# JiaruiFeng/KP-GNN

Hardware: AMD Instinct MI355X
Metric: graphs/sec KP-GIN fwd+bwd, ZINC-12k K=8 L=8 h=104 (higher is better)
Workload: dtype f32; 1 GPU; ZINC-12k-shaped synthetic molecules, KPGINPlus K=8 L=8 h=104 kernel=spd geometric combine, fwd+bwd+Adam, L1 loss; global_batch=2048, nodes_per_batch=47450, khop_edges_per_batch=1018372, active_pairs_per_batch=1018372, parallelism=dp1, launch=hipGraph replay of fwd+bwd, batches=4 pre-staged batches cycled

## Files before the change

### include/kpgnn.h

```cpp
#ifndef KPGNN_H_
#define KPGNN_H_

#include <stddef.h>
#include <stdint.h>

#ifdef __cplusplus
extern "C" {
#endif

#define KPGNN_ABI_VERSION 1

#define KPGNN_OK 0
#define KPGNN_EINVAL (-1)
#define KPGNN_EHIP (-2)
#define KPGNN_ELIMIT (-3)

typedef void* kpgnn_stream_t;

int kpgnn_abi_version(void);
const char* kpgnn_last_error(void);

int kpgnn_device_info(int* cu_count, int* lds_bytes_per_block, int* wavefront, char* arch, int arch_len);


// ... 44 lines not shown
    int32_t* rowptr_dst; int32_t* col_dst; uint16_t* code_dst;
    int32_t* rowptr_src; int32_t* col_src; uint16_t* code_src;
    int64_t* batch;
    int32_t* node_src;
    int32_t nodes_per_tile; int32_t* tile_ptr; uint32_t* tile_pack;
    int32_t* ent_node_ptr;
    int32_t num_prefix; int32_t* prefix_ptr; uint32_t* prefix_pack; int32_t* prefix_scratch;
    int32_t n_node_rows; kpgnn_row_gather node_rows[8];
    int32_t n_graph_rows; kpgnn_row_gather graph_rows[8];
} kpgnn_collate_desc;

int kpgnn_collate(const kpgnn_collate_desc* d, kpgnn_stream_t stream);

int kpgnn_regression_loss(const float* score, const float* y, int64_t n, int32_t kind, float* loss, float* dscore,
                          kpgnn_stream_t stream);

int kpgnn_score_head_fwd(const float* pooled, const float* w, const float* bias, int64_t G, int32_t D, float* score,
                         kpgnn_stream_t stream);
int kpgnn_score_head_bwd(const float* pooled, const float* w, const float* dscore, int64_t G, int32_t D, float* dpooled,
                         float* dw, float* db, kpgnn_stream_t stream);

int kpgnn_adam_step(float* param, const float* grad, float* exp_avg, float* exp_avg_sq, int64_t n, int64_t step,
                    double lr, double beta1, double beta2, double eps, double weight_decay, kpgnn_stream_t stream);

int kpgnn_adam_step_device(float* param, const float* grad, float* exp_avg, float* exp_avg_sq, int64_t n, int64_t* state,
                           double lr, double beta1, double beta2, double eps, double weight_decay, kpgnn_stream_t stream);

int kpgnn_multi_copy(int32_t count, const float* const* src, float* const* dst, const int64_t* numel, kpgnn_stream_t stream);

typedef struct kpgnn_reduce_job {
    const float* slab; int32_t nslab; int64_t elems;
    float* out[4]; int64_t n_out[4];
} kpgnn_reduce_job;
int kpgnn_reduce_jobs(const kpgnn_reduce_job* jobs, int32_t count, kpgnn_stream_t stream);

enum { KPGNN_STORE_F32 = 0, KPGNN_STORE_BF16 = 1 };

enum { KPGNN_MATH_AUTO = 0, KPGNN_MATH_F32 = 1 };

enum {
    KPGNN_MODE_GIN = 0,
    KPGNN_MODE_GINPLUS = 1,
    KPGNN_MODE_GCN = 2,
    KPGNN_MODE_SUM = 3
};

typedef struct kpgnn_agg_fwd_desc {
    int32_t N, K, D;
    int32_t K_csr;
    int32_t mode;
    int32_t n_code0, n_codek;
    int32_t use_tables;
    const int32_t* rowptr;
    const int32_t* col;
    const uint16_t* code;
    const float* dis;
    const float* x;
    int64_t x_sn, x_sk;
    const float* table0;
    const float* tablek;
    const float* periph;
    int64_t p_sn, p_sk;
    const float* eps;
    float* out;
    int64_t o_sn, o_sk;
    float* pre;
    const float* theta;
    float* hout;
    const float* xbias;
    const float* ptab;
    const int32_t* uid;
    int64_t uid_stride;
    const float* x_slot[16];
    int32_t n_dict;
    const float* alphas;
    int32_t storage;
    const int32_t* n_dyn;
    const int32_t* graph_ptr; int32_t num_graphs; int32_t max_graph_nodes;
    const float* hinit;
    const float* hinit2;
} kpgnn_agg_fwd_desc;

int kpgnn_aggregate_fwd(const kpgnn_agg_fwd_desc* d, kpgnn_stream_t stream);

typedef struct kpgnn_agg_bwd_desc {
    int32_t N, K, D, K_csr, mode, n_code0, n_codek, use_tables;
    const int32_t* rowptr_src;
    const int32_t* col_src;
    const uint16_t* code_src;
    const float* dis;
    const float* g;
    int64_t g_sn, g_sk;
    const float* eps;
    float* gx;
    int64_t gx_sn, gx_sk;
    float* gtable0;
    float* gtablek;
    float* gx_slot[16];
    uint32_t accumulate_mask;
    int32_t storage;
    const int32_t* n_dyn;
} kpgnn_agg_bwd_desc;

int kpgnn_aggregate_bwd(const kpgnn_agg_bwd_desc* d, kpgnn_stream_t stream);

typedef struct kpgnn_table_grad_desc {
    int32_t N, K, D, nodes_per_tile, n_code0, n_codek;
    int32_t n_dict, dict_src;
    const int32_t* tile_ptr;
    const uint32_t* tile_pack;
    const float* g;
    int64_t g_sn, g_sk;
    const int32_t* uid;
    int64_t uid_stride;
    const float* theta;
    const float* gh;
    float* gtable0;
    float* gtablek;
    float* gdict;
    void* workspace;
    size_t workspace_bytes;
    int32_t kernel;
    const uint32_t* dict_pack;
    int32_t dict_pack_K;
    const float* extra_slab;
    int32_t extra_nslab;
    int64_t extra_elems;
    float* extra_out;
    int32_t storage;
    const float* fuse_pre;
    const float* fuse_ptab;
    const int32_t* fuse_uid;
    int64_t fuse_uid_stride;
    int32_t fuse_n_dict;
    float* fuse_g;
    float* fuse_gtheta;
    const float* fuse_alphas;
    float* fuse_galphas;
    void* fuse_workspace;
    size_t fuse_workspace_bytes;
    int32_t accumulate_dict;
    const kpgnn_reduce_job* pending;
    const int32_t* n_dyn;
    int32_t max_multiplicity;
} kpgnn_table_grad_desc;

size_t kpgnn_table_grad_workspace_bytes(int32_t N, int32_t K, int32_t D, int32_t nodes_per_tile,
                                        int32_t n_code0, int32_t n_codek, int32_t n_dict);
int kpgnn_table_grad(const kpgnn_table_grad_desc* d, kpgnn_stream_t stream);
size_t kpgnn_table_grad_fuse_workspace_bytes(int32_t K, int32_t D);
int kpgnn_dict_tile_pack(const int32_t* uid, int64_t uid_stride, int32_t N, int32_t K, int32_t nodes_per_tile,
                         uint32_t* pack, kpgnn_stream_t stream);

typedef struct kpgnn_dict_grad_desc {
    int32_t N, K, D, n_dict;
    const int32_t* uid;
    int64_t uid_stride;
    const float* theta;
    const float* gh;
    float* gdict;
    void* workspace;
    size_t workspace_bytes;
    int32_t defer_reduce;
    const int32_t* dominant;
    const int32_t* n_dyn;
} kpgnn_dict_grad_desc;
// ... 289 lines not shown
```

### kp_gnn_amd/_lib.py

```python
import ctypes
import os

_PKG = os.path.dirname(os.path.abspath(__file__))
HIP_LIB_PATH = os.path.join(_PKG, "libkpgnn_hip.so")

MODE_GIN, MODE_GINPLUS, MODE_GCN, MODE_SUM = 0, 1, 2, 3

c_i32, c_i64, c_f32p, c_vp = ctypes.c_int32, ctypes.c_int64, ctypes.c_void_p, ctypes.c_void_p


MATH_AUTO, MATH_F32 = 0, 1
DENSE_MATH = MATH_AUTO


class KpgnnError(RuntimeError):
    pass


class AggFwdDesc(ctypes.Structure):
    _fields_ = [
        ("N", c_i32), ("K", c_i32), ("D", c_i32), ("K_csr", c_i32), ("mode", c_i32),
        ("n_code0", c_i32), ("n_codek", c_i32), ("use_tables", c_i32),
        ("rowptr", c_vp), ("col", c_vp), ("code", c_vp), ("dis", c_vp),
        ("x", c_vp), ("x_sn", c_i64), ("x_sk", c_i64),
# ... 184 lines not shown
        ("math", c_i32), ("workspace", c_vp), ("workspace_bytes", ctypes.c_size_t),
    ]

    def __init__(self, *a, **kw):
        super().__init__(*a, **kw)
        self.math = DENSE_MATH


class HopMlpDesc(ctypes.Structure):
    _fields_ = [
        ("N", c_i64), ("K", c_i32), ("DI", c_i32), ("DO", c_i32), ("H", c_i32),
        ("s", c_vp), ("w1", c_vp), ("b1", c_vp), ("w2", c_vp), ("b2", c_vp), ("theta", c_vp),
        ("wc", c_vp), ("bc", c_vp), ("h1", c_vp), ("h2", c_vp), ("out", c_vp), ("gout", c_vp), ("gs", c_vp), ("gflat", c_vp),
        ("workspace", c_vp), ("workspace_bytes", ctypes.c_size_t),
    ]


class TgsDesc(ctypes.Structure):
    _fields_ = [
        ("M", c_i64), ("C", c_i32), ("D", c_i32), ("R", c_i32),
        ("idx", c_vp), ("col_offset", c_vp), ("table", c_vp), ("bias", c_vp),
        ("out", c_vp), ("out_stride", c_i64), ("gout", c_vp), ("gout_stride", c_i64), ("gtable", c_vp),
        ("workspace", c_vp), ("workspace_bytes", ctypes.c_size_t),
        ("n_dyn", c_vp),
    ]


class EncTablesDesc(ctypes.Structure):
    _fields_ = [
        ("H", c_i32), ("num_components", c_i32), ("num_encoders", c_i32),
        ("comp_emb", c_vp * 16), ("comp_rows", c_i32 * 16), ("comp_encoder", c_i32 * 16),
        ("enc_w", c_vp * 4), ("enc_b", c_vp * 4), ("enc_gate", c_vp * 4), ("enc_mult", ctypes.c_float * 4),
        ("enc_squash", c_i32 * 4),
        ("table", c_vp), ("pre", c_vp), ("bias", c_vp), ("gtable", c_vp), ("gbias", c_vp),
        ("comp_gemb", c_vp * 16), ("enc_gw", c_vp * 4), ("enc_gb", c_vp * 4), ("enc_ggate", c_vp * 4),
    ]


class PoolDesc(ctypes.Structure):
    _fields_ = [
        ("N", c_i64), ("G", c_i32), ("D", c_i32), ("mode", c_i32),
        ("graph_ptr", c_vp), ("batch", c_vp), ("x", c_vp), ("x_stride", c_i64), ("out", c_vp),
        ("gout", c_vp), ("gx", c_vp), ("gx_stride", c_i64),
        ("n_dyn", c_vp),
    ]


class DatasetView(ctypes.Structure):
    _fields_ = [
        ("K", c_i32), ("G", c_i32), ("node_ptr", c_vp), ("pair_ptr", c_vp), ("ent_ptr", c_vp),
        ("rowptr_dst", c_vp), ("rowptr_src", c_vp), ("col_dst", c_vp), ("col_src", c_vp),
        ("code_dst", c_vp), ("code_src", c_vp), ("ent_rel", c_vp), ("ent", c_vp),
    ]


class RowGather(ctypes.Structure):
    _fields_ = [("src", c_vp), ("dst", c_vp), ("row_bytes", c_i32)]


class CollateDesc(ctypes.Structure):
    _fields_ = [
        ("ds", DatasetView), ("B", c_i32), ("N", c_i32), ("A", c_i64), ("n_ent", c_i64), ("hdr", c_vp),
        ("rowptr_dst", c_vp), ("col_dst", c_vp), ("code_dst", c_vp),
        ("rowptr_src", c_vp), ("col_src", c_vp), ("code_src", c_vp),
        ("batch", c_vp), ("node_src", c_vp),
        ("nodes_per_tile", c_i32), ("tile_ptr", c_vp), ("tile_pack", c_vp), ("ent_node_ptr", c_vp),
        ("num_prefix", c_i32), ("prefix_ptr", c_vp), ("prefix_pack", c_vp), ("prefix_scratch", c_vp),
        ("n_node_rows", c_i32), ("node_rows", RowGather * 8),
        ("n_graph_rows", c_i32), ("graph_rows", RowGather * 8),
    ]


SIGNATURES = {
    "kpgnn_abi_version": (ctypes.c_int, []),
    "kpgnn_last_error": (ctypes.c_char_p, []),
    "kpgnn_device_info": (ctypes.c_int, [ctypes.POINTER(ctypes.c_int)] * 3 + [ctypes.c_char_p, ctypes.c_int]),
    "kpgnn_csr_stats": (ctypes.c_int, [c_vp, c_i64, c_vp, c_i64, c_i64, c_i32, c_vp, c_vp]),
    "kpgnn_csr_workspace_bytes": (ctypes.c_size_t, [c_i64, c_i64, c_i64, c_i32]),
    "kpgnn_csr_build": (ctypes.c_int, [c_vp, c_i64, c_vp, c_i64, c_i64, c_i32, c_i64, c_i64,
                                       c_vp, c_vp, c_vp, c_vp, c_vp, c_vp, c_i32, c_vp, c_vp,
                                       c_vp, ctypes.c_size_t, c_vp]),
    "kpgnn_aggregate_fwd": (ctypes.c_int, [ctypes.POINTER(AggFwdDesc), c_vp]),
    "kpgnn_aggregate_bwd": (ctypes.c_int, [ctypes.POINTER(AggBwdDesc), c_vp]),
    "kpgnn_table_grad_workspace_bytes": (ctypes.c_size_t, [c_i32] * 7),
    "kpgnn_table_grad": (ctypes.c_int, [ctypes.POINTER(TableGradDesc), c_vp]),
    "kpgnn_table_grad_fuse_workspace_bytes": (ctypes.c_size_t, [c_i32, c_i32]),
    "kpgnn_dict_grad_workspace_bytes": (ctypes.c_size_t, [c_i32] * 4),
    "kpgnn_dict_grad": (ctypes.c_int, [ctypes.POINTER(DictGradDesc), c_vp]),
    "kpgnn_dict_grad_multi": (ctypes.c_int, [ctypes.POINTER(DictGradMultiDesc), c_vp]),
    "kpgnn_dict_grad_slabs": (c_i32, [c_i32]),
    "kpgnn_tile_pack_filter": (ctypes.c_int, [c_vp, c_vp, c_i64, c_i32, c_vp, c_vp, c_vp, c_vp]),
    "kpgnn_tile_pack_prefixes": (ctypes.c_int, [c_vp, c_vp, c_i64, c_i32, c_i64, c_vp, c_vp, c_vp, c_vp, c_i32, c_vp]),
    "kpgnn_collate": (ctypes.c_int, [ctypes.POINTER(CollateDesc), c_vp]),
    "kpgnn_regression_loss": (ctypes.c_int, [c_vp, c_vp, c_i64, c_i32, c_vp, c_vp, c_vp]),
    "kpgnn_score_head_fwd": (ctypes.c_int, [c_vp, c_vp, c_vp, c_i64, c_i32, c_vp, c_vp]),
    "kpgnn_score_head_bwd": (ctypes.c_int, [c_vp, c_vp, c_vp, c_i64, c_i32, c_vp, c_vp, c_vp, c_vp]),
    "kpgnn_adam_step": (ctypes.c_int, [c_vp, c_vp, c_vp, c_vp, c_i64, c_i64, ctypes.c_double, ctypes.c_double, ctypes.c_double,
                                       ctypes.c_double, ctypes.c_double, c_vp]),
    "kpgnn_reduce_jobs": (ctypes.c_int, [c_vp, c_i32, c_vp]),
    "kpgnn_adam_step_device": (ctypes.c_int, [c_vp, c_vp, c_vp, c_vp, c_i64, c_vp, ctypes.c_double, ctypes.c_double,
                                              ctypes.c_double, ctypes.c_double, ctypes.c_double, c_vp]),
    "kpgnn_multi_copy": (ctypes.c_int, [c_i32, c_vp, c_vp, c_vp, c_vp]),
    "kpgnn_dict_tile_pack": (ctypes.c_int, [c_vp, c_i64, c_i32, c_i32, c_i32, c_vp, c_vp]),
    "kpgnn_combine_bwd_workspace_bytes": (ctypes.c_size_t, [c_i32] * 3),
    "kpgnn_combine_bwd": (ctypes.c_int, [ctypes.POINTER(CombineBwdDesc), c_vp]),
    "kpgnn_bn_fwd": (ctypes.c_int, [ctypes.POINTER(BnDesc), c_vp]),
    "kpgnn_bn_bwd": (ctypes.c_int, [ctypes.POINTER(BnBwdDesc), c_vp]),
    "kpgnn_wgrad_workspace_bytes": (ctypes.c_size_t, [c_i32, c_i32]),
    "kpgnn_linear_wgrad": (ctypes.c_int, [ctypes.POINTER(WgradDesc), c_vp]),
    "kpgnn_linear_wgrad_pair": (ctypes.c_int, [ctypes.POINTER(WgradDesc), ctypes.POINTER(WgradDesc), c_vp]),
    "kpgnn_wgrad_group_workspace_bytes": (ctypes.c_size_t, [c_i32, c_i32, c_i32]),
    "kpgnn_linear_wgrad_group": (ctypes.c_int, [ctypes.POINTER(WgradDesc), c_vp, c_i32, c_vp]),
    "kpgnn_linear_bn": (ctypes.c_int, [ctypes.POINTER(LinearBnDesc), c_vp]),
    "kpgnn_enc_tables_fwd": (ctypes.c_int, [ctypes.POINTER(EncTablesDesc), c_vp]),
    "kpgnn_enc_tables_bwd": (ctypes.c_int, [ctypes.POINTER(EncTablesDesc), c_vp]),
    "kpgnn_segment_pool_fwd": (ctypes.c_int, [ctypes.POINTER(PoolDesc), c_vp]),
    "kpgnn_segment_pool_bwd": (ctypes.c_int, [ctypes.POINTER(PoolDesc), c_vp]),
    "kpgnn_stat_slot_bytes": (ctypes.c_size_t, [c_i32]),
    "kpgnn_stream_capture_id": (ctypes.c_int, [c_vp, ctypes.POINTER(ctypes.c_uint64)]),
    "kpgnn_attn_fwd": (ctypes.c_int, [ctypes.POINTER(AttnDesc), c_vp]),
    "kpgnn_attn_bwd": (ctypes.c_int, [ctypes.POINTER(AttnDesc), c_vp]),
    "kpgnn_attn_scan_fwd": (ctypes.c_int, [ctypes.POINTER(AttnScanDesc), c_vp]),
    "kpgnn_attn_scan_bwd": (ctypes.c_int, [ctypes.POINTER(AttnScanDesc), c_vp]),
    "kpgnn_attn_scan_unpad": (ctypes.c_int, [c_vp, c_vp, c_vp, c_vp, c_vp, c_vp, c_i32, c_i32, c_vp]),
    "kpgnn_linear_fwd": (ctypes.c_int, [ctypes.POINTER(LinearDesc), c_vp]),
    "kpgnn_linear_split_workspace_bytes": (ctypes.c_size_t, [c_i32, c_i32, c_i32]),
    "kpgnn_linear_split_many": (ctypes.c_int, [ctypes.POINTER(SplitJob), c_i32, c_vp]),
    "kpgnn_linear_group_fwd": (ctypes.c_int, [ctypes.POINTER(LinearGroupDesc), c_vp]),
    "kpgnn_geo_theta_fwd": (ctypes.c_int, [c_vp, c_i32, c_i32, c_vp, c_vp]),
    "kpgnn_geo_theta_bwd": (ctypes.c_int, [c_vp, c_vp, c_vp, c_i32, c_i32, c_vp, c_vp]),
    "kpgnn_hop_mlp_workspace_bytes": (ctypes.c_size_t, [c_i64, c_i32, c_i32, c_i32, c_i32]),
    "kpgnn_hop_mlp_fwd": (ctypes.c_int, [ctypes.POINTER(HopMlpDesc), c_vp]),
    "kpgnn_hop_mlp_bwd": (ctypes.c_int, [ctypes.POINTER(HopMlpDesc), c_vp]),
    "kpgnn_table_gather_sum_fwd": (ctypes.c_int, [ctypes.POINTER(TgsDesc), c_vp]),
    "kpgnn_table_gather_sum_bwd": (ctypes.c_int, [ctypes.POINTER(TgsDesc), c_vp]),
    "kpgnn_table_gather_sum_bwd_workspace_bytes": (ctypes.c_size_t, [c_i64, c_i32, c_i32]),
}

_lib = None


def load(path=None):
    global _lib
    if _lib is not None and path is None:
        return _lib
    path = path or HIP_LIB_PATH
    if not os.path.exists(path):
        raise KpgnnError(
            f"{path} not found: the HIP extension is required (no CPU fallback). "
            "Build it with `python -m kp_gnn_amd.build` (or __graft_entry__.build()).")
    try:
        lib = ctypes.CDLL(path)
    except OSError as e:
        raise KpgnnError(f"cannot load {path}: {e}") from e
    for name, (res, args) in SIGNATURES.items():
        fn = getattr(lib, name)
        fn.restype = res
        fn.argtypes = args
    if lib.kpgnn_abi_version() != 1:
        raise KpgnnError("libkpgnn_hip.so ABI version mismatch")
    _lib = lib
    return lib


def check(rc, what):
    if rc != 0:
# ... 3 lines not shown
```

### kp_gnn_amd/csrc/aggregate.hip

```cpp
#include <initializer_list>

#include "kpgnn_common.h"

namespace kpgnn {
namespace {

constexpr int kBlock = 256;
constexpr int kMaxLdsTableBytes = 96 * 1024;

template <int VEC> struct Vec;
template <> struct Vec<1> { using T = float; };
template <> struct Vec<2> { using T = float2; };
template <> struct Vec<4> { using T = float4; };

template <int VEC> struct V {
    float v[VEC];
    __device__ __forceinline__ static V zero() { V r; for (int i = 0; i < VEC; ++i) r.v[i] = 0.f; return r; }
    __device__ __forceinline__ static V load(const float* p) {
        V r;
        typename Vec<VEC>::T t = *reinterpret_cast<const typename Vec<VEC>::T*>(p);
        const float* f = reinterpret_cast<const float*>(&t);
        for (int i = 0; i < VEC; ++i) r.v[i] = f[i];
        return r;
    }
// ... 567 lines not shown
    const int nb = resident_blocks(agg_bwd_kernel<VEC, G, GCN, TAB, BF, GXACC>, kBlock, lds);
    const unsigned grid = pick_grid(tiles, nb > 0 ? nb : 4);
    hipLaunchKernelGGL((agg_bwd_kernel<VEC, G, GCN, TAB, BF, GXACC>), dim3(grid), dim3(kBlock), lds, s, p);
    KPGNN_LAUNCH_CHECK("agg_bwd_kernel");
    return KPGNN_OK;
}

template <int VEC, int G>
int launch_bwd_mode(const BwdParams& p, int tab, size_t lds, hipStream_t s) {
    const bool gcn = p.mode == KPGNN_MODE_GCN;
    if (p.bf) {
        if constexpr (VEC == 4) {
            if (!gcn && tab == 0 && p.mode != KPGNN_MODE_GIN) return launch_bwd<VEC, G, false, 0, true>(p, 0, s);
        }
        return fail(KPGNN_EINVAL, "aggregate_bwd: bf16 storage needs mode GINPLUS/SUM without table gradients and D %% 4 == 0");
    }
    if (p.gx && p.acc_mask) {
        if (!gcn && tab == 0) return launch_bwd<VEC, G, false, 0, false, true>(p, 0, s);
        return fail(KPGNN_EINVAL, "aggregate_bwd: accumulate_mask with gx needs a non-GCN mode without table gradients");
    }
    switch (tab) {
        case 0: return gcn ? launch_bwd<VEC, G, true, 0>(p, 0, s) : launch_bwd<VEC, G, false, 0>(p, 0, s);
        case 1: return gcn ? launch_bwd<VEC, G, true, 1>(p, lds, s) : launch_bwd<VEC, G, false, 1>(p, lds, s);
        default: return gcn ? launch_bwd<VEC, G, true, 2>(p, 0, s) : launch_bwd<VEC, G, false, 2>(p, 0, s);
    }
}

#define KP_DISPATCH_SHAPE(CALL)                                                                    \
    switch (vec * 100 + g) {                                                                       \
        case 404: return CALL(4, 4); case 408: return CALL(4, 8); case 416: return CALL(4, 16);    \
        case 432: return CALL(4, 32); case 464: return CALL(4, 64);                                \
        case 204: return CALL(2, 4); case 208: return CALL(2, 8); case 216: return CALL(2, 16);    \
        case 232: return CALL(2, 32); case 264: return CALL(2, 64);                                \
        case 104: return CALL(1, 4); case 108: return CALL(1, 8); case 116: return CALL(1, 16);    \
        case 132: return CALL(1, 32); case 164: return CALL(1, 64);                                \
    }

}
}

using namespace kpgnn;

extern "C" int kpgnn_aggregate_fwd(const kpgnn_agg_fwd_desc* d, kpgnn_stream_t stream) {
    KPGNN_REQUIRE(d != nullptr, "aggregate_fwd: NULL descriptor");
    KPGNN_REQUIRE(d->N >= 0 && d->K >= 1 && d->D >= 1 && d->K_csr >= d->K, "aggregate_fwd: bad N=%d K=%d D=%d K_csr=%d",
                  d->N, d->K, d->D, d->K_csr);
    if ((int64_t)d->N * d->K_csr >= ((int64_t)1 << 31)) return fail(KPGNN_ELIMIT, "aggregate_fwd: N*K exceeds int32");
    if (d->N == 0) return KPGNN_OK;
    KPGNN_REQUIRE(d->rowptr != nullptr, "aggregate_fwd: NULL rowptr");
    if (!d->x) {
        KPGNN_REQUIRE(d->K <= 16, "aggregate_fwd: per-hop inputs need K <= 16");
        for (int k = 0; k < d->K; ++k) KPGNN_REQUIRE(d->x_slot[k] != nullptr, "aggregate_fwd: NULL x and NULL x_slot[%d]", k);
    }
    KPGNN_REQUIRE(d->mode >= KPGNN_MODE_GIN && d->mode <= KPGNN_MODE_SUM, "aggregate_fwd: unknown mode %d", d->mode);
    KPGNN_REQUIRE(d->mode != KPGNN_MODE_GCN || d->dis, "aggregate_fwd: GCN mode needs dis");
    const bool combine = d->theta != nullptr;
    KPGNN_REQUIRE(combine ? d->hout != nullptr : d->out != nullptr, "aggregate_fwd: NULL output");
    KPGNN_REQUIRE(!d->alphas || combine, "aggregate_fwd: alphas needs the theta buffer it fills");
    int tab = 0;
    size_t lds = 0;
    if (d->use_tables)
        KPGNN_REQUIRE(d->table0 && d->n_code0 >= 1 && (d->K == 1 || (d->tablek && d->n_codek >= 1)),
                      "aggregate_fwd: missing embedding tables");
    KPGNN_REQUIRE(d->periph || !d->uid || (d->ptab && d->uid_stride >= d->K), "aggregate_fwd: dictionary P needs ptab and uid_stride >= K");
    if (d->use_tables) {
        KPGNN_REQUIRE(d->mode != KPGNN_MODE_GCN || (d->n_code0 >= 2 && (d->K == 1 || d->n_codek >= 2)),
                      "aggregate_fwd: GCN needs code row 1 (self loop) in both tables");
        lds = sizeof(float) * (size_t)d->D * ((size_t)d->n_code0 + (size_t)(d->K > 1 ? d->n_codek : 0));
        tab = lds <= (size_t)kMaxLdsTableBytes ? 1 : 2;
    }
    {
        bool handled = false;
        const int rc = agg_lds_fwd(d, (hipStream_t)stream, &handled);
        if (rc != KPGNN_OK || handled) return rc;
    }
    KPGNN_REQUIRE((!d->hinit && !d->hinit2) || (combine && !d->alphas), "aggregate_fwd: hinit / hinit2 need a fused combine with a given theta");
    if (!d->hinit && !d->hinit2) {
        bool handled = false;
        int rc = d->n_dyn ? KPGNN_OK : agg_narrow_fwd(d, (hipStream_t)stream, &handled);
        if (rc != KPGNN_OK || handled) return rc;
        if (!d->n_dyn) rc = agg_small_fwd(d, (hipStream_t)stream, &handled);
        if (rc != KPGNN_OK || handled) return rc;
    }
    FwdParams p;
    p.lds_theta = p.lds_ptab = 0;
    if (tab == 1) {
        lds = (lds + 15) & ~(size_t)15;
        const size_t cap = 36 * 1024;
        const size_t th_b = combine ? sizeof(float) * (size_t)d->K * d->D : 0;
        if (th_b && lds + th_b <= cap) { p.lds_theta = d->K * d->D; lds += (th_b + 15) & ~(size_t)15; }
        const size_t pt_b = (!d->periph && d->ptab && d->n_dict > 0) ? sizeof(float) * (size_t)d->n_dict * d->D : 0;
        if (pt_b && lds + pt_b <= cap) { p.lds_ptab = d->n_dict * d->D; lds += (pt_b + 15) & ~(size_t)15; }
    }
    p.N = d->N; p.n_dyn = d->n_dyn; p.K = d->K; p.D = d->D; p.K_csr = d->K_csr; p.n_code0 = d->n_code0; p.n_codek = d->K > 1 ? d->n_codek : 0;
    p.mode = d->mode; p.combine = combine ? 1 : 0; p.bf = d->storage == KPGNN_STORE_BF16 ? 1 : 0;
    KPGNN_REQUIRE(d->storage == KPGNN_STORE_F32 || d->storage == KPGNN_STORE_BF16, "aggregate_fwd: unknown storage %d", d->storage);
    p.rowptr = d->rowptr; p.col = d->col; p.code = d->code; p.dis = d->dis;
    p.x = d->x; p.x_sn = d->x_sn; p.x_sk = d->x_sk;
    p.table0 = d->table0; p.tablek = d->tablek;
    p.periph = d->periph; p.p_sn = d->p_sn; p.p_sk = d->p_sk;
    p.eps = d->eps; p.out = d->out; p.o_sn = d->o_sn; p.o_sk = d->o_sk; p.pre = d->pre; p.theta = d->theta; p.hout = d->hout; p.hinit = d->hinit; p.hinit2 = d->hinit2; p.xbias = d->xbias;
    p.alphas = nullptr; p.theta_out = nullptr;
    if (d->alphas) {
        if (p.lds_theta) { p.alphas = d->alphas; p.theta_out = const_cast<float*>(d->theta); }
        else {
            const int rc = geo_theta_fwd_launch(d->alphas, d->K, d->D, const_cast<float*>(d->theta), (hipStream_t)stream);
            if (rc != KPGNN_OK) return rc;
        }
    }
    p.ptab = d->periph ? nullptr : d->ptab; p.uid = d->periph ? nullptr : d->uid; p.uid_stride = d->uid_stride;
    KPGNN_REQUIRE(p.uid == nullptr || (p.ptab != nullptr && p.uid_stride >= d->K), "aggregate_fwd: dictionary P needs ptab and uid_stride >= K");
    uintptr_t slot_bits = 0;
    for (int k = 0; k < 16; ++k) {
        p.xs[k] = (!d->x && k < d->K) ? d->x_slot[k] : nullptr;
        slot_bits |= (uintptr_t)p.xs[k] & 15;
    }
    const void* slot_align = (const void*)(slot_bits | 16);
    if ((uint64_t)d->N * (uint64_t)d->x_sn * 4u >= (1ull << 32))
        return fail(KPGNN_ELIMIT, "aggregate_fwd: N * x row stride = %lld floats exceeds the 32-bit byte offsets of the gather", (long long)d->N * d->x_sn);
    const int vec = pick_vec(d->D, {d->x ? (const void*)d->x : slot_align, d->periph, d->out, d->pre, d->table0, d->tablek, d->theta, d->hout, d->hinit, d->hinit2, d->xbias, d->periph ? nullptr : d->ptab},
                             {d->x_sn, d->x ? d->x_sk : 0, d->periph ? d->p_sn : 0, d->periph ? d->p_sk : 0,
                              d->out ? d->o_sn : 0, d->out ? d->o_sk : 0});
    const int lanes = (d->D + vec - 1) / vec;
    if (lanes > 64) return fail(KPGNN_ELIMIT, "aggregate_fwd: D=%d with %d-wide access needs %d lanes > 64", d->D, vec, lanes);
    const int g = pick_group(lanes);
    hipStream_t s = (hipStream_t)stream;
#define KP_CALL(VEC_, G_) launch_fwd_mode<VEC_, G_>(p, tab, lds, s)
    KP_DISPATCH_SHAPE(KP_CALL)
#undef KP_CALL
    return fail(KPGNN_EINVAL, "aggregate_fwd: no kernel for vec=%d g=%d", vec, g);
}

extern "C" int kpgnn_aggregate_bwd(const kpgnn_agg_bwd_desc* d, kpgnn_stream_t stream) {
    KPGNN_REQUIRE(d != nullptr, "aggregate_bwd: NULL descriptor");
    KPGNN_REQUIRE(d->N >= 0 && d->K >= 1 && d->D >= 1 && d->K_csr >= d->K, "aggregate_bwd: bad N=%d K=%d D=%d K_csr=%d",
                  d->N, d->K, d->D, d->K_csr);
    if ((int64_t)d->N * d->K_csr >= ((int64_t)1 << 31)) return fail(KPGNN_ELIMIT, "aggregate_bwd: N*K exceeds int32");
    if (d->N == 0) return KPGNN_OK;
    KPGNN_REQUIRE(d->rowptr_src && d->g, "aggregate_bwd: NULL rowptr/g");
    if (!d->gx) {
        KPGNN_REQUIRE(d->K <= 16, "aggregate_bwd: per-hop outputs need K <= 16");
        for (int k = 0; k < d->K; ++k) KPGNN_REQUIRE(d->gx_slot[k] != nullptr, "aggregate_bwd: NULL gx and NULL gx_slot[%d]", k);
    }
    KPGNN_REQUIRE(d->mode >= KPGNN_MODE_GIN && d->mode <= KPGNN_MODE_SUM, "aggregate_bwd: unknown mode %d", d->mode);
    KPGNN_REQUIRE(d->mode != KPGNN_MODE_GCN || d->dis, "aggregate_bwd: GCN mode needs dis");
    int tab = 0;
    size_t lds = 0;
    if (d->use_tables && d->gtable0) {
        KPGNN_REQUIRE(d->n_code0 >= 1 && (d->K == 1 || (d->gtablek && d->n_codek >= 1)), "aggregate_bwd: missing table grads");
        lds = sizeof(float) * (size_t)d->D * ((size_t)d->n_code0 + (size_t)(d->K > 1 ? d->n_codek : 0));
        tab = lds <= (size_t)kMaxLdsTableBytes ? 1 : 2;
    }
    {
        bool handled = false;
        const int rc = d->n_dyn ? KPGNN_OK : agg_narrow_bwd(d, (hipStream_t)stream, &handled);
        if (rc != KPGNN_OK || handled) return rc;
    }
    BwdParams p;
    p.N = d->N; p.n_dyn = d->n_dyn; p.K = d->K; p.D = d->D; p.K_csr = d->K_csr; p.n_code0 = d->n_code0; p.n_codek = d->K > 1 ? d->n_codek : 0;
    p.mode = d->mode; p.bf = d->storage == KPGNN_STORE_BF16 ? 1 : 0;
    KPGNN_REQUIRE(d->storage == KPGNN_STORE_F32 || d->storage == KPGNN_STORE_BF16, "aggregate_bwd: unknown storage %d", d->storage);
    p.rowptr = d->rowptr_src; p.col = d->col_src; p.code = d->code_src; p.dis = d->dis;
    p.g = d->g; p.g_sn = d->g_sn; p.g_sk = d->g_sk; p.eps = d->eps;
    p.gx = d->gx; p.gx_sn = d->gx_sn; p.gx_sk = d->gx_sk; p.gtable0 = d->gtable0; p.gtablek = d->gtablek;
    uintptr_t slot_bits = 0;
    for (int k = 0; k < 16; ++k) {
// ... 28 lines not shown
```

### kp_gnn_amd/csrc/kpgnn_common.h

```cpp
#pragma once
#include <hip/hip_runtime.h>

#include <cstdarg>
#include <cstdint>
#include <cstdio>

#include "kpgnn.h"

namespace kpgnn {

char* error_buffer();

inline int fail(int code, const char* fmt, ...) {
    va_list ap;
    va_start(ap, fmt);
    vsnprintf(error_buffer(), 512, fmt, ap);
    va_end(ap);
    return code;
}

#define KPGNN_HIP_TRY(expr)                                                                      \
    do {                                                                                         \
        hipError_t e_ = (expr);                                                                  \
        if (e_ != hipSuccess)                                                                    \
// ... 31 lines not shown
const DeviceFacts& device_facts();

hipError_t ensure_dynamic_lds(const void* func, size_t bytes);
size_t linear3_workspace_bytes(int O, int I, int group);
int linear3_group_fwd(const kpgnn_linear_group_desc* d, hipStream_t s, bool* handled);
int linear3_blocked(const kpgnn_linear_desc* d, hipStream_t s, bool* handled);
int linear3_split_w(const float* w, int64_t wn, int64_t wk, int O, int I, void* frag, hipStream_t s);

struct ThetaFinish {
    const float* slab; int nslab;
    const float* alpha; const float* theta; int K, D;
    float* gtheta; float* galpha;
};
int slab_reduce(const float* slab, int nslab, int64_t elems, float* out0, int64_t n0, float* out1, int64_t n1,
                float* out2, hipStream_t s, int64_t n2 = 0, float* out3 = nullptr, const float* slab_b = nullptr,
                int nslab_b = 0, int64_t elems_b = 0, float* out_b = nullptr, const ThetaFinish* tf = nullptr,
                int acc_mask = 0,
                const kpgnn_reduce_job* pending = nullptr);

__device__ __forceinline__ void theta_finish_block(const ThetaFinish& f, int blk, float* sm) {
    float (*part)[65] = reinterpret_cast<float (*)[65]>(sm);
    float* tot = sm + 16 * 65;
    float* ths = tot + 64;
    const int K = f.K, D = f.D, CB = 64 / K;
    const int o = threadIdx.x & 63, slice = threadIdx.x >> 6;
    const int k = o / CB, cq = o - k * CB;
    const int d = blk * CB + cq;
    const bool ok = k < K && cq < CB && d < D;
    const int64_t KD = (int64_t)K * D, e = (int64_t)k * D + d;
    float th_mine = 0.f, al_mine = 0.f;
    if (slice == 0 && ok) th_mine = f.theta[e];
    const bool colthread = threadIdx.x < CB && blk * CB + threadIdx.x < D;
    if (colthread && f.galpha) al_mine = f.alpha[blk * CB + threadIdx.x];
    float s = 0.f;
    if (ok) {
        int b = slice;
        for (; b + 48 < f.nslab; b += 64) {
            const float v0 = f.slab[(int64_t)b * KD + e], v1 = f.slab[(int64_t)(b + 16) * KD + e];
            const float v2 = f.slab[(int64_t)(b + 32) * KD + e], v3 = f.slab[(int64_t)(b + 48) * KD + e];
            s += v0; s += v1; s += v2; s += v3;
        }
        for (; b < f.nslab; b += 16) s += f.slab[(int64_t)b * KD + e];
    }
    part[slice][o] = s;
    __syncthreads();
    if (slice == 0) {
        float t = 0.f;
#pragma unroll
        for (int q = 0; q < 16; ++q) t += part[q][o];
        tot[o] = t;
        ths[o] = th_mine;
        if (ok) f.gtheta[e] = t;
    }
    __syncthreads();
    if (colthread && f.galpha) {
        const int c = threadIdx.x, dd = blk * CB + c;
        const float a = 1.0f / (1.0f + __expf(-al_mine));
        const float q = 1.0f - a;
        float dot = 0.f;
        for (int kk = 0; kk < K; ++kk) dot = fmaf(ths[kk * CB + c], tot[kk * CB + c], dot);
        float acc = 0.f, pw = 1.0f, pwm1 = 0.f;
        for (int kk = 0; kk < K; ++kk) {
            const float dt = ths[kk * CB + c] * (tot[kk * CB + c] - dot);
            acc = fmaf(dt, pw - (float)kk * a * pwm1, acc);
            pwm1 = pw;
            pw *= q;
        }
        f.galpha[dd] = a * q * acc;
    }
}

int geo_theta_fwd_launch(const float* alpha, int K, int D, float* theta, hipStream_t s);
int gtheta_finish_launch(const float* slab, int nslab, const float* alpha, const float* theta, int K, int D, float* gtheta,
                         float* galpha, hipStream_t s);

int table_grad_mfma(const kpgnn_table_grad_desc* d, hipStream_t s, bool* handled);
size_t table_grad_mfma_ws_bytes(int N, int K, int D, int NT, int n0, int nk, int U);

int agg_narrow_fwd(const kpgnn_agg_fwd_desc* d, hipStream_t s, bool* handled);
int agg_narrow_bwd(const kpgnn_agg_bwd_desc* d, hipStream_t s, bool* handled);
int agg_lds_fwd(const kpgnn_agg_fwd_desc* d, hipStream_t s, bool* handled);
int agg_small_fwd(const kpgnn_agg_fwd_desc* d, hipStream_t s, bool* handled);
int agg_small_bwd(const kpgnn_agg_bwd_desc* d, hipStream_t s, bool* handled);

__device__ __forceinline__ float fast_erf(float z, float* e2_out) {
    const float az = fabsf(z);
    const float t = __builtin_amdgcn_rcpf(fmaf(0.3275911f, az, 1.0f));
    float poly = 1.061405429f;
    poly = fmaf(poly, t, -1.453152027f);
    poly = fmaf(poly, t, 1.421413741f);
    poly = fmaf(poly, t, -0.284496736f);
    poly = fmaf(poly, t, 0.254829592f);
    const float e2 = __expf(-az * az);
    *e2_out = e2;
    return copysignf(fmaf(-poly * t, e2, 1.0f), z);
}

__device__ __forceinline__ uint32_t f32_to_bf16_bits(float f) {
    const uint32_t u = __float_as_uint(f);
    return (u + 0x7FFFu + ((u >> 16) & 1u)) >> 16;
}
template <int VEC> __device__ __forceinline__ void ld_bf16(const void* q, float (&v)[VEC]) {
    if (VEC == 4) {
        const uint2 t = *reinterpret_cast<const uint2*>(q);
        v[0] = __uint_as_float(t.x << 16); v[1 % VEC] = __uint_as_float(t.x & 0xFFFF0000u);
        v[2 % VEC] = __uint_as_float(t.y << 16); v[3 % VEC] = __uint_as_float(t.y & 0xFFFF0000u);
    } else if (VEC == 2) {
        const uint32_t t = *reinterpret_cast<const uint32_t*>(q);
        v[0] = __uint_as_float(t << 16); v[1 % VEC] = __uint_as_float(t & 0xFFFF0000u);
    } else {
        v[0] = __uint_as_float((uint32_t)*reinterpret_cast<const uint16_t*>(q) << 16);
    }
}
template <int VEC> __device__ __forceinline__ void ld_bf16_stream(const void* q, float (&v)[VEC]) {
    if (VEC == 4) {
        const uint32_t* w = reinterpret_cast<const uint32_t*>(q);
        const uint32_t x = __builtin_nontemporal_load(w), y = __builtin_nontemporal_load(w + 1);
        v[0] = __uint_as_float(x << 16); v[1 % VEC] = __uint_as_float(x & 0xFFFF0000u);
        v[2 % VEC] = __uint_as_float(y << 16); v[3 % VEC] = __uint_as_float(y & 0xFFFF0000u);
    } else {
        ld_bf16<VEC>(q, v);
    }
}
template <int VEC> __device__ __forceinline__ void st_bf16_stream(void* q, const float (&v)[VEC]) {
    if (VEC == 4) {
        uint32_t* w = reinterpret_cast<uint32_t*>(q);
        __builtin_nontemporal_store(f32_to_bf16_bits(v[0]) | (f32_to_bf16_bits(v[1 % VEC]) << 16), w);
        __builtin_nontemporal_store(f32_to_bf16_bits(v[2 % VEC]) | (f32_to_bf16_bits(v[3 % VEC]) << 16), w + 1);
    } else if (VEC == 2) {
        __builtin_nontemporal_store(f32_to_bf16_bits(v[0]) | (f32_to_bf16_bits(v[1 % VEC]) << 16), reinterpret_cast<uint32_t*>(q));
    } else {
        *reinterpret_cast<uint16_t*>(q) = (uint16_t)f32_to_bf16_bits(v[0]);
    }
}
template <int VEC> __device__ __forceinline__ void st_bf16(void* q, const float (&v)[VEC]) {
    if (VEC == 4) {
        uint2 t;
        t.x = f32_to_bf16_bits(v[0]) | (f32_to_bf16_bits(v[1 % VEC]) << 16);
        t.y = f32_to_bf16_bits(v[2 % VEC]) | (f32_to_bf16_bits(v[3 % VEC]) << 16);
        *reinterpret_cast<uint2*>(q) = t;
    } else if (VEC == 2) {
        *reinterpret_cast<uint32_t*>(q) = f32_to_bf16_bits(v[0]) | (f32_to_bf16_bits(v[1 % VEC]) << 16);
    } else {
        *reinterpret_cast<uint16_t*>(q) = (uint16_t)f32_to_bf16_bits(v[0]);
    }
}

struct XcdTileWalk {
    int64_t cur, end, step;
    __device__ XcdTileWalk(int64_t num_tiles) {
        const int64_t b = blockIdx.x, g = gridDim.x;
        if (g < kNumXcd || (g % kNumXcd) != 0) {
            cur = b; end = num_tiles; step = g;
            return;
        }
        const int64_t xcd = b % kNumXcd, slot = b / kNumXcd, nslot = g / kNumXcd;
        const int64_t per = (num_tiles + kNumXcd - 1) / kNumXcd;
        const int64_t lo = xcd * per;
        int64_t hi = lo + per;
        if (hi > num_tiles) hi = num_tiles;
        cur = lo + slot; end = hi; step = nslot;
    }
    __device__ bool valid() const { return cur < end; }
    __device__ void next() { cur += step; }
};

// ... 17 lines not shown
```

Before: 639,800 graphs/s.

## Add direct-to-LDS gather kernel for fused aggregate forward

Adds a new forward aggregation kernel that gathers neighbour feature rows straight into a per-wave LDS ring with global_load_lds, then reduces them with the code tables, GELU, peripheral table and theta combine fused in. It also prefetches the next node's rowptr/col/code metadata while the current gather is in flight. The aim is to cut register-staged gather latency and VGPR pressure for the k-hop sum. The cost is one block per CU with heavy LDS use, full vmcnt waits per chunk, and a dispatch path that is tried only after the existing LDS, narrow and small paths decline.

```diff
diff --git a/include/kpgnn.h b/include/kpgnn.h
--- a/include/kpgnn.h
+++ b/include/kpgnn.h
@@ -150,6 +150,8 @@
 } kpgnn_agg_fwd_desc;
 
 int kpgnn_aggregate_fwd(const kpgnn_agg_fwd_desc* d, kpgnn_stream_t stream);
+
+int kpgnn_set_gather_dma(int enable);
 
 typedef struct kpgnn_agg_bwd_desc {
     int32_t N, K, D, K_csr, mode, n_code0, n_codek, use_tables;
diff --git a/kp_gnn_amd/_lib.py b/kp_gnn_amd/_lib.py
--- a/kp_gnn_amd/_lib.py
+++ b/kp_gnn_amd/_lib.py
@@ -290,6 +290,7 @@
                                        c_vp, ctypes.c_size_t, c_vp]),
     "kpgnn_aggregate_fwd": (ctypes.c_int, [ctypes.POINTER(AggFwdDesc), c_vp]),
     "kpgnn_aggregate_bwd": (ctypes.c_int, [ctypes.POINTER(AggBwdDesc), c_vp]),
+    "kpgnn_set_gather_dma": (ctypes.c_int, [c_i32]),
     "kpgnn_table_grad_workspace_bytes": (ctypes.c_size_t, [c_i32] * 7),
     "kpgnn_table_grad": (ctypes.c_int, [ctypes.POINTER(TableGradDesc), c_vp]),
     "kpgnn_table_grad_fuse_workspace_bytes": (ctypes.c_size_t, [c_i32, c_i32]),
diff --git a/kp_gnn_amd/csrc/aggregate.hip b/kp_gnn_amd/csrc/aggregate.hip
--- a/kp_gnn_amd/csrc/aggregate.hip
+++ b/kp_gnn_amd/csrc/aggregate.hip
@@ -673,6 +673,11 @@
         if (!d->n_dyn) rc = agg_small_fwd(d, (hipStream_t)stream, &handled);
         if (rc != KPGNN_OK || handled) return rc;
     }
+    {
+        bool handled = false;
+        const int rc = agg_dma_fwd(d, (hipStream_t)stream, &handled);
+        if (rc != KPGNN_OK || handled) return rc;
+    }
     FwdParams p;
     p.lds_theta = p.lds_ptab = 0;
     if (tab == 1) {
diff --git a/kp_gnn_amd/csrc/aggregate_dma.hip b/kp_gnn_amd/csrc/aggregate_dma.hip
--- /dev/null
+++ b/kp_gnn_amd/csrc/aggregate_dma.hip
@@ -0,0 +1,336 @@
+#include <initializer_list>
+
+#include "kpgnn_common.h"
+
+namespace kpgnn {
+namespace {
+
+constexpr int kDmaWaves = 16;
+constexpr int kDmaBlock = kDmaWaves * kWave;
+constexpr int kPieceBytes = 1024;
+constexpr int kMinPieces = 4;
+constexpr int kMaxPieces = 16;
+
+int g_gather_dma = 1;
+
+typedef __attribute__((address_space(3))) void* lds_void_ptr;
+typedef __attribute__((address_space(1))) void* global_void_ptr;
+
+struct DmaParams {
+    const int32_t* n_dyn;
+    int N, K, D, K_csr, n_code0, n_codek, n_dict, pieces;
+    const int32_t* rowptr;
+    const int32_t* col;
+    const uint16_t* code;
+    const float* x; int64_t x_sn, x_sk;
+    const float* xs[16];
+    const float* table0;
+    const float* tablek;
+    float* pre;
+    const float* theta;
+    const float* alphas;
+    float* theta_out;
+    float* hout;
+    const float* hinit;
+    const float* hinit2;
+    const float* xbias;
+    const float* ptab; const int32_t* uid; int64_t uid_stride;
+};
+
+struct F4 {
+    float v[4];
+    __device__ __forceinline__ static F4 zero() { F4 r; for (int q = 0; q < 4; ++q) r.v[q] = 0.f; return r; }
+    __device__ __forceinline__ static F4 load(const float* p) {
+        const float4 t = *reinterpret_cast<const float4*>(p);
+        F4 r; r.v[0] = t.x; r.v[1] = t.y; r.v[2] = t.z; r.v[3] = t.w;
+        return r;
+    }
+    __device__ __forceinline__ void store_stream(float* p) const {
+        for (int q = 0; q < 4; ++q) __builtin_nontemporal_store(v[q], p + q);
+    }
+    __device__ __forceinline__ void add(const F4& o) { for (int q = 0; q < 4; ++q) v[q] += o.v[q]; }
+    __device__ __forceinline__ void fma(float s, const F4& o) { for (int q = 0; q < 4; ++q) v[q] = fmaf(s, o.v[q], v[q]); }
+};
+
+__device__ __forceinline__ float gelu_exact(float x) {
+    float e2;
+    return 0.5f * x * (1.0f + fast_erf(x * 0.70710678118654752440f, &e2));
+}
+
+template <bool FAST>
+__global__ void __launch_bounds__(kDmaBlock, 1)
+agg_dma_kernel(const DmaParams p) {
+    const int N_live = live_rows(p.N, p.n_dyn);
+    const int D = p.D, K = p.K;
+    extern __shared__ __attribute__((aligned(16))) float lds[];
+    const int n0 = FAST ? p.n_code0 * D : 0, nk = FAST ? p.n_codek * D : 0;
+    float* th_l = lds + ((n0 + nk + 3) & ~3);
+    float* pt_l = th_l + ((K * D + 3) & ~3);
+    uint64_t* hb_l = reinterpret_cast<uint64_t*>(pt_l + (FAST ? ((p.n_dict * D + 3) & ~3) : 0));
+    char* ring = reinterpret_cast<char*>(hb_l + 16);
+    if (FAST) {
+        for (int t = threadIdx.x; t < n0; t += kDmaBlock) lds[t] = p.table0[t];
+        for (int t = threadIdx.x; t < nk; t += kDmaBlock) lds[n0 + t] = p.tablek[t];
+        for (int t = threadIdx.x; t < p.n_dict * D; t += kDmaBlock) pt_l[t] = p.ptab[t];
+    }
+    if (FAST && p.alphas) {
+        for (int d = threadIdx.x; d < D; d += kDmaBlock) {
+            const float a = 1.0f / (1.0f + __expf(-p.alphas[d]));
+            const float q = 1.0f - a;
+            float pw = 1.0f, mx = -INFINITY;
+            for (int k = 0; k < K; ++k) { mx = fmaxf(mx, a * pw); pw *= q; }
+            float sum = 0.f;
+            pw = 1.0f;
+            for (int k = 0; k < K; ++k) { sum += __expf(a * pw - mx); pw *= q; }
+            const float inv = 1.0f / sum;
+            pw = 1.0f;
+            for (int k = 0; k < K; ++k) {
+                const float th = __expf(a * pw - mx) * inv;
+                th_l[k * D + d] = th;
+                if (blockIdx.x == 0) p.theta_out[(int64_t)k * D + d] = th;
+                pw *= q;
+            }
+        }
+    } else {
+        for (int t = threadIdx.x; t < K * D; t += kDmaBlock) th_l[t] = p.theta[t];
+    }
+    if (threadIdx.x == 0)
+        for (int t = 0; t < K; ++t) hb_l[t] = (uint64_t)(uintptr_t)(p.x ? p.x + (int64_t)t * p.x_sk : p.xs[t]);
+    __syncthreads();
+
+    const int wave = threadIdx.x / kWave;
+    const int lane = threadIdx.x & (kWave - 1);
+    const int sg = lane >> 5, sl = lane & 31, sg_lane0 = lane - sl;
+    const int C = D >> 2;
+    const bool col_ok = sl < C;
+    const int c0 = col_ok ? sl * 4 : 0;
+    const uint32_t lane_c = col_ok ? (uint32_t)sl : 0u;
+    const uint32_t inv_c = (65536u + (uint32_t)C - 1u) / (uint32_t)C;
+    const int cap_pairs = min(32, (p.pieces * 32) / C);
+    const uint32_t xrow_b = (uint32_t)p.x_sn * 4u, trow_b = (uint32_t)D * 4u;
+    const uint32_t lane_b = (uint32_t)c0 * 4u;
+    char* wring = ring + (size_t)wave * p.pieces * kPieceBytes;
+    const char* my_ring = wring + sg * 512;
+    auto ring_row = [&](uint32_t g) {
+        return reinterpret_cast<const float*>(my_ring + (g >> 5) * kPieceBytes + (g & 31u) * 16u);
+    };
+    const float* tab0 = lds;
+    const float* tabk = lds + n0;
+
+    const int64_t num_tiles = ((int64_t)N_live + 1) / 2;
+    int64_t cur, end, step;
+    {
+        const int64_t b = blockIdx.x, g = gridDim.x;
+        if (g < kNumXcd || (g % kNumXcd) != 0) {
+            cur = b * kDmaWaves + wave; end = num_tiles; step = g * kDmaWaves;
+        } else {
+            const int64_t xcd = b % kNumXcd, slot = (b / kNumXcd) * kDmaWaves + wave, nslot = (g / kNumXcd) * kDmaWaves;
+            const int64_t per = (num_tiles + kNumXcd - 1) / kNumXcd;
+            const int64_t lo = xcd * per;
+            end = lo + per < num_tiles ? lo + per : num_tiles;
+            cur = lo + slot; step = nslot;
+        }
+    }
+
+    int myrp = 0, myuid = 0, mycol = 0, mycode = 0;
+    bool have_w0 = false;
+    if (cur < end && cur * 2 + sg < N_live) {
+        const int64_t i = cur * 2 + sg;
+        myrp = p.rowptr[i * p.K_csr + (sl <= K ? sl : K)];
+        if (FAST) myuid = p.uid[i * p.uid_stride + (sl < K ? sl : 0)];
+    }
+    for (; cur < end; cur += step) {
+        const int64_t i = cur * 2 + sg;
+        if (i >= N_live) continue;
+        const int64_t i_next = (cur + step) * 2 + sg;
+        const bool has_next = cur + step < end && i_next < N_live;
+        int nrp = 0, nuid = 0, ncol = 0, ncode = 0;
+        bool next_meta = false, next_w0 = false;
+        F4 hsum = F4::zero();
+        if (!FAST && p.hinit) hsum = F4::load(p.hinit + i * (int64_t)D + c0);
+        if (!FAST && p.hinit2) hsum.add(F4::load(p.hinit2 + i * (int64_t)D + c0));
+        const int beg_all = __shfl(myrp, sg_lane0);
+        const int end_all = __shfl(myrp, sg_lane0 + K);
+
+        int k = 0;
+        int seg_beg = beg_all;
+        int seg_end = __shfl(myrp, sg_lane0 + 1);
+        F4 acc = F4::zero();
+        int wb = beg_all - 32;
+        uint32_t a_lo = 0, a_hi = 0, ctab = 0;
+        int cb = beg_all;
+        while (true) {
+            int n = 0;
+            if (cb < end_all) {
+                if (cb >= wb + 32) {
+                    const bool first = cb == beg_all;
+                    wb = cb;
+                    const int idx = wb + sl;
+                    int hop = 0;
+                    for (int kk = 1; kk < K; ++kk) hop += idx >= __shfl(myrp, sg_lane0 + kk) ? 1 : 0;
+                    int cv = mycol, cd = mycode;
+                    if (!(first && have_w0)) {
+                        cv = 0; cd = 0;
+                        if (idx < end_all) { cv = p.col[idx]; if (FAST) cd = p.code[idx]; }
+                    }
+                    a_lo = a_hi = ctab = 0;
+                    if (idx < end_all) {
+                        const uint64_t a = hb_l[hop] + (uint64_t)((uint32_t)cv * xrow_b);
+                        a_lo = (uint32_t)a; a_hi = (uint32_t)(a >> 32);
+                        ctab = (uint32_t)cd * trow_b;
+                    }
+                }
+                n = min(cap_pairs, min(end_all, wb + 32) - cb);
+                asm volatile("s_waitcnt lgkmcnt(0)" ::: "memory");
+                const uint32_t nchunks = (uint32_t)(n * C);
+                const int npieces = (int)((nchunks + 31u) >> 5);
+                const int pbase = cb - wb;
+#pragma unroll 4
+                for (int q = 0; q < npieces; ++q) {
+                    const uint32_t g = (uint32_t)q * 32u + (uint32_t)sl;
+                    const uint32_t pl = (g * inv_c) >> 16;
+                    const uint32_t c = g - pl * (uint32_t)C;
+                    const int src_lane = sg_lane0 + min(pbase + (int)pl, 31);
+                    const uint32_t lo = (uint32_t)__shfl((int)a_lo, src_lane);
+                    const uint32_t hi = (uint32_t)__shfl((int)a_hi, src_lane);
+                    if (g < nchunks) {
+                        const char* src = reinterpret_cast<const char*>(((uint64_t)hi << 32) | lo) + c * 16u;
+                        __builtin_amdgcn_global_load_lds((global_void_ptr)src, (lds_void_ptr)(wring + q * kPieceBytes), 16, 0, 0);
+                    }
+                }
+                if (!next_meta && has_next) {
+                    nrp = p.rowptr[i_next * p.K_csr + (sl <= K ? sl : K)];
+                    if (FAST) nuid = p.uid[i_next * p.uid_stride + (sl < K ? sl : 0)];
+                    next_meta = true;
+                }
+                asm volatile("s_waitcnt vmcnt(0)" ::: "memory");
+                if (next_meta && !next_w0) {
+                    const int nb = __shfl(nrp, sg_lane0), ne = __shfl(nrp, sg_lane0 + K);
+                    if (nb + sl < ne) { ncol = p.col[nb + sl]; if (FAST) ncode = p.code[nb + sl]; }
+                    next_w0 = true;
+                }
+            }
+            const int bend = cb + n;
+            int pos = cb;
+            while (true) {
+                const int lim = min(seg_end, bend);
+                const char* tabb = reinterpret_cast<const char*>(k == 0 ? tab0 : tabk);
+                for (; pos + 1 < lim; pos += 2) {
+                    const uint32_t g0 = (uint32_t)((pos - cb) * C) + lane_c;
+                    F4 r0 = F4::load(ring_row(g0));
+                    F4 r1 = F4::load(ring_row(g0 + (uint32_t)C));
+                    if (FAST) {
+                        const uint32_t t0 = (uint32_t)__shfl((int)ctab, sg_lane0 + (pos - wb));
+                        const uint32_t t1 = (uint32_t)__shfl((int)ctab, sg_lane0 + (pos + 1 - wb));
+                        r0.add(F4::load(reinterpret_cast<const float*>(tabb + (t0 + lane_b))));
+                        r1.add(F4::load(reinterpret_cast<const float*>(tabb + (t1 + lane_b))));
+                    }
+                    acc.add(r0);
+                    acc.add(r1);
+                }
+                if (pos < lim) {
+                    F4 r0 = F4::load(ring_row((uint32_t)((pos - cb) * C) + lane_c));
+                    if (FAST) {
+                        const uint32_t t0 = (uint32_t)__shfl((int)ctab, sg_lane0 + (pos - wb));
+                        r0.add(F4::load(reinterpret_cast<const float*>(tabb + (t0 + lane_b))));
+                    }
+                    acc.add(r0);
+                    ++pos;
+                }
+                if (pos < seg_end) break;
+                const int uk = FAST ? __shfl(myuid, sg_lane0 + k) : 0;
+                if (col_ok) {
+                    F4 v = acc;
+                    if (p.xbias != nullptr && k >= 1) v.fma((float)(seg_end - seg_beg), F4::load(p.xbias + c0));
+                    if (FAST) {
+                        v.store_stream(p.pre + (i * K + k) * (int64_t)D + c0);
+                        for (int q = 0; q < 4; ++q) v.v[q] = gelu_exact(v.v[q]);
+                        v.add(F4::load(pt_l + (int64_t)uk * D + c0));
+                    }
+                    const F4 th = F4::load(th_l + k * D + c0);
+                    for (int q = 0; q < 4; ++q) hsum.v[q] = fmaf(th.v[q], v.v[q], hsum.v[q]);
+                }
+                acc = F4::zero();
+                if (++k == K) break;
+                seg_beg = seg_end;
+                seg_end = __shfl(myrp, sg_lane0 + k + 1);
+            }
+            if (k == K) break;
+            cb = bend;
+        }
+        if (col_ok) hsum.store_stream(p.hout + i * (int64_t)D + c0);
+        if (has_next && !next_meta) {
+            nrp = p.rowptr[i_next * p.K_csr + (sl <= K ? sl : K)];
+            if (FAST) nuid = p.uid[i_next * p.uid_stride + (sl < K ? sl : 0)];
+        }
+        myrp = nrp; myuid = nuid; mycol = ncol; mycode = ncode; have_w0 = next_w0;
+    }
+}
+
+bool al16(const void* q) { return ((uintptr_t)q & 15) == 0; }
+
+}
+
+int agg_dma_fwd(const kpgnn_agg_fwd_desc* d, hipStream_t s, bool* handled) {
+    *handled = false;
+    if (!g_gather_dma || d->N < 4096 || d->storage != KPGNN_STORE_F32 || d->D % 4 || d->D > 128 || d->K > 16) return KPGNN_OK;
+    if (!d->theta || !d->hout || d->periph || d->mode == KPGNN_MODE_GCN) return KPGNN_OK;
+    const bool fast = d->mode == KPGNN_MODE_GINPLUS && d->use_tables && d->table0 && (d->K == 1 || d->tablek) && d->uid &&
+                      d->ptab && d->n_dict > 0 && d->uid_stride >= d->K && d->pre && !d->hinit && !d->hinit2;
+    const bool pull = d->mode == KPGNN_MODE_SUM && !d->use_tables && !d->uid && !d->pre && !d->alphas;
+    if (!fast && !pull) return KPGNN_OK;
+    if (d->x_sn % 4 || (d->x && (d->x_sk % 4 || !al16(d->x)))) return KPGNN_OK;
+    if (!d->x)
+        for (int k = 0; k < d->K; ++k)
+            if (!al16(d->x_slot[k])) return KPGNN_OK;
+    for (const void* q : {(const void*)d->theta, (const void*)d->hout, (const void*)d->hinit, (const void*)d->hinit2,
+                          (const void*)d->xbias, (const void*)d->pre, (const void*)d->ptab, (const void*)d->table0,
+                          (const void*)d->tablek})
+        if (q && !al16(q)) return KPGNN_OK;
+    if ((uint64_t)d->N * (uint64_t)d->x_sn * 4u >= (1ull << 32)) return KPGNN_OK;
+    const int n_codek = fast && d->K > 1 ? d->n_codek : 0;
+    auto up4 = [](size_t f) { return (f + 3) & ~(size_t)3; };
+    const size_t side = sizeof(float) * (up4(fast ? (size_t)(d->n_code0 + n_codek) * d->D : 0) + up4((size_t)d->K * d->D) +
+                                         (fast ? up4((size_t)d->n_dict * d->D) : 0)) + 16 * sizeof(uint64_t);
+    const size_t lds_cap = (size_t)device_facts().lds_per_block;
+    if (side + (size_t)kDmaWaves * kMinPieces * kPieceBytes > lds_cap) return KPGNN_OK;
+    int pieces = (int)((lds_cap - side) / ((size_t)kDmaWaves * kPieceBytes));
+    if (pieces > kMaxPieces) pieces = kMaxPieces;
+    const size_t lds = side + (size_t)kDmaWaves * pieces * kPieceBytes;
+
+    const void* fn = fast ? (const void*)agg_dma_kernel<true> : (const void*)agg_dma_kernel<false>;
+    KPGNN_HIP_TRY(ensure_dynamic_lds(fn, lds));
+    const int nb = fast ? resident_blocks(agg_dma_kernel<true>, kDmaBlock, lds) : resident_blocks(agg_dma_kernel<false>, kDmaBlock, lds);
+    if (nb < 1) return KPGNN_OK;
+
+    DmaParams p;
+    p.n_dyn = d->n_dyn; p.N = d->N; p.K = d->K; p.D = d->D; p.K_csr = d->K_csr;
+    p.n_code0 = fast ? d->n_code0 : 0; p.n_codek = n_codek; p.n_dict = fast ? d->n_dict : 0; p.pieces = pieces;
+    p.rowptr = d->rowptr; p.col = d->col; p.code = d->code;
+    p.x = d->x; p.x_sn = d->x_sn; p.x_sk = d->x_sk;
+    for (int k = 0; k < 16; ++k) p.xs[k] = (!d->x && k < d->K) ? d->x_slot[k] : nullptr;
+    p.table0 = fast ? d->table0 : nullptr; p.tablek = fast ? d->tablek : nullptr;
+    p.pre = fast ? d->pre : nullptr;
+    p.theta = d->theta; p.alphas = fast ? d->alphas : nullptr; p.theta_out = const_cast<float*>(d->theta);
+    p.hout = d->hout; p.hinit = d->hinit; p.hinit2 = d->hinit2; p.xbias = d->xbias;
+    p.ptab = fast ? d->ptab : nullptr; p.uid = fast ? d->uid : nullptr; p.uid_stride = d->uid_stride;
+
+    const int64_t tiles = ((int64_t)d->N + 1) / 2;
+    int64_t blocks = (tiles + kDmaWaves - 1) / kDmaWaves;
+    const int64_t cap = (int64_t)device_facts().cu_count * nb;
+    if (blocks > cap) blocks = cap;
+    if (blocks >= kNumXcd) blocks = blocks / kNumXcd * kNumXcd;
+    if (fast) hipLaunchKernelGGL((agg_dma_kernel<true>), dim3((unsigned)blocks), dim3(kDmaBlock), lds, s, p);
+    else hipLaunchKernelGGL((agg_dma_kernel<false>), dim3((unsigned)blocks), dim3(kDmaBlock), lds, s, p);
+    KPGNN_LAUNCH_CHECK("agg_dma_kernel");
+    *handled = true;
+    return KPGNN_OK;
+}
+
+}
+
+extern "C" int kpgnn_set_gather_dma(int enable) {
+    const int old = kpgnn::g_gather_dma;
+    kpgnn::g_gather_dma = enable ? 1 : 0;
+    return old;
+}
diff --git a/kp_gnn_amd/csrc/kpgnn_common.h b/kp_gnn_amd/csrc/kpgnn_common.h
--- a/kp_gnn_amd/csrc/kpgnn_common.h
+++ b/kp_gnn_amd/csrc/kpgnn_common.h
@@ -137,6 +137,7 @@
 int agg_lds_fwd(const kpgnn_agg_fwd_desc* d, hipStream_t s, bool* handled);
 int agg_small_fwd(const kpgnn_agg_fwd_desc* d, hipStream_t s, bool* handled);
 int agg_small_bwd(const kpgnn_agg_bwd_desc* d, hipStream_t s, bool* handled);
+int agg_dma_fwd(const kpgnn_agg_fwd_desc* d, hipStream_t s, bool* handled);
 
 __device__ __forceinline__ float fast_erf(float z, float* e2_out) {
     const float az = fabsf(z);
```

Result: slower. 616,500 graphs/s, median of 2 (-3.6%).
